# bupt-cist/vqa-playground-pytorch

Measured on AMD Instinct MI355X. Metric: VQA samples/sec (fwd+bwd), CoR2 batch 512, 36x2048 regions, higher is better.
Workload: dtype f32

## Files before the change

vqa_playground_pytorch_amd/csrc/bilinear_dw_rt.hip:

```cpp
#include <cstdlib>

#include "bilinear_folded.hpp"
#include "gemm_f32_rt.hpp"

namespace vqa {

namespace {

constexpr int kSpans = 5;
constexpr int kCols = 64 * kSpans;
typedef float f32x2 __attribute__((ext_vector_type(2)));
typedef unsigned int u32x2 __attribute__((__vector_size__(2 * sizeof(unsigned int))));

struct DwRtArgs {
  const float* g;
  const float* x;
  const float* h2;
  const float* w[2];
  const float* b[2];
  float* slab;
  float* dbslab;
  float* part;
  int B, N, L, H;
  int HB;
  int spl;
  unsigned long long* stamps;
};

template <int R, int NS, int D, int TUNE = 0>
__global__ __launch_bounds__(rt::kThreads, 1) void bilinear_dw_rt_kernel(DwRtArgs p) {
  using rt::f32x4;
  extern __shared__ __attribute__((aligned(16))) char smem_raw[];
  float* Ws = reinterpret_cast<float*>(smem_raw);
  const int tid = threadIdx.x, lane = tid & 63, r = lane & 15, gq = lane >> 4;
  const int wave = __builtin_amdgcn_readfirstlane(tid >> 6);
  const int eh = wave & 1, sl = wave >> 1;
  const int id = xcd_remap(blockIdx.x, gridDim.x);
  const int hb = id % p.HB, sg = id / p.HB;
  const int h0 = hb * 16;
  unsigned long long tk_in = 0;
  if constexpr ((TUNE & 4) != 0) tk_in = __builtin_amdgcn_s_memrealtime();
  const int slice = sg * 2 + sl;
  const int b_lo = min(slice * p.spl, p.B), b_hi = min(p.B, b_lo + p.spl);
  const int L = p.L, H = p.H, N = p.N;

  const rt::rsrc_t Gb = rt::make_rsrc(p.g, (size_t)p.B * N * H * 4);
  const rt::rsrc_t Xb = rt::make_rsrc(p.x, (size_t)p.B * N * L * 4);
  const rt::rsrc_t Hb = rt::make_rsrc(p.h2, (size_t)p.B * R * H * 4);
  const uint32_t offG = ((uint32_t)gq * (uint32_t)H + (uint32_t)min(h0 + r, H - 1)) * 4u;
  uint32_t offX[kSpans];
#pragma unroll
  for (int q = 0; q < kSpans; ++q) offX[q] = ((uint32_t)gq * (uint32_t)L + (uint32_t)(64 * q + 4 * r + 2 * eh)) * 4u;
  const uint32_t offH = (uint32_t)(h0 + 4 * gq) * 4u;
  const bool one_lane = (r == (L % 64) / 4) && (eh == (L % 4) / 2);

  f32x4 acc[R][kSpans][2];
#pragma unroll
  for (int rk = 0; rk < R; ++rk)
#pragma unroll
    for (int q = 0; q < kSpans; ++q)
#pragma unroll
      for (int e = 0; e < 2; ++e) acc[rk][q][e] = f32x4{0.f, 0.f, 0.f, 0.f};

  struct Step {
    float a;
    f32x2 xb[kSpans];
  };
  const int row_hi = b_hi * N;
  auto load_step = [&](Step& st, int row) {
    const uint32_t rw = (uint32_t)min(row, max(row_hi - 4, 0));
    st.a = rt::ldg4(Gb, offG, rw * (uint32_t)H * 4u);
#pragma unroll
    for (int q = 0; q < kSpans; ++q)
      st.xb[q] = __builtin_bit_cast(f32x2, __builtin_amdgcn_raw_buffer_load_b64(Xb, (int)offX[q], (int)(rw * (uint32_t)L * 4u), 0));
  };
  auto fix_ones = [&](Step& st) {
    const float v0 = st.xb[kSpans - 1][0], v1 = st.xb[kSpans - 1][1];
    st.xb[kSpans - 1][0] = one_lane ? 1.f : v0;
    st.xb[kSpans - 1][1] = one_lane ? 0.f : v1;
  };

  Step ring[D];
#pragma unroll
  for (int d = 0; d < D; ++d) load_step(ring[d], b_lo * N + 4 * d);
  f32x4 h2v[R];
#pragma unroll
  for (int rk = 0; rk < R; ++rk) h2v[rk] = rt::ldg16(Hb, offH, (uint32_t)((min(b_lo, p.B - 1) * R + rk) * H) * 4u);

  {
    const int hl = tid >> 4, c0 = (tid & 15) * 2;
    const int h = h0 + hl;
    f32x2 wv[R][kCols / 32];
    float bv[R];
    constexpr uint32_t kOut = 0x80000000u;
#pragma unroll
    for (int rk = 0; rk < R; ++rk) {
      const rt::rsrc_t Wb = rt::make_rsrc(p.w[rk], (size_t)H * L * 4);
      const rt::rsrc_t Bb = rt::make_rsrc(p.b[rk], (size_t)H * 4);
      bv[rk] = rt::ldg4(Bb, h < H ? (uint32_t)h * 4u : kOut, 0u);
#pragma unroll
      for (int k = 0; k < kCols / 32; ++k) {
        const int col = c0 + 32 * k;
        const uint32_t off = (h < H && col < L) ? ((uint32_t)h * (uint32_t)L + (uint32_t)col) * 4u : kOut;
        wv[rk][k] = __builtin_bit_cast(f32x2, __builtin_amdgcn_raw_buffer_load_b64(Wb, (int)off, 0, 0));
      }
    }
#pragma unroll
    for (int rk = 0; rk < R; ++rk)
#pragma unroll
      for (int k = 0; k < kCols / 32; ++k)
        if (c0 + 32 * k == L) wv[rk][k][0] = bv[rk];
#pragma unroll
    for (int rk = 0; rk < R; ++rk)
#pragma unroll
      for (int k = 0; k < kCols / 32; ++k)
        *reinterpret_cast<f32x2*>(Ws + (rk * 16 + hl) * kCols + c0 + 32 * k) = wv[rk][k];
  }
  __syncthreads();

  if (b_lo < b_hi) {

    f32x4 P[kSpans][2];
    unsigned long long cyc_steps = 0, cyc_fold = 0, tk0 = 0;
    if constexpr ((TUNE & 4) != 0) tk0 = __builtin_amdgcn_s_memrealtime();
    for (int b = b_lo; b < b_hi; ++b) {
      const int row0 = b * N;
      unsigned long long c0 = 0, c1 = 0;
      if constexpr ((TUNE & 4) != 0) c0 = __builtin_amdgcn_s_memtime();
      f32x4 h2n[R];
#pragma unroll
      for (int rk = 0; rk < R; ++rk) h2n[rk] = rt::ldg16(Hb, offH, (uint32_t)((min(b + 1, b_hi - 1) * R + rk) * H) * 4u);
#pragma unroll
      for (int s = 0; s < NS; ++s) {
        static_assert(NS % D == 0, "a ring slot must mean the same step in every sample");
        Step& st = ring[s % D];
        fix_ones(st);
#pragma unroll
        for (int q = 0; q < kSpans; ++q)
#pragma unroll
          for (int e = 0; e < 2; ++e)
            P[q][e] = __builtin_amdgcn_mfma_f32_16x16x4f32(st.a, st.xb[q][e], s == 0 ? f32x4{0.f, 0.f, 0.f, 0.f} : P[q][e], 0, 0, 0);
        load_step(ring[(s + D - 1) % D], row0 + 4 * (s - 1 + D));
        __builtin_amdgcn_sched_group_barrier(0x002, 2, 0);
        __builtin_amdgcn_sched_group_barrier(0x008, 1, 0);
#pragma unroll
        for (int t = 0; t < kSpans + 1; ++t) {
          __builtin_amdgcn_sched_group_barrier(0x020, 1, 0);
          __builtin_amdgcn_sched_group_barrier(0x008, 1, 0);
        }
        __builtin_amdgcn_sched_group_barrier(0x008, 2 * kSpans - 1 - (kSpans + 1), 0);
        __builtin_amdgcn_sched_barrier(0);
      }
      if constexpr ((TUNE & 4) != 0) {
        c1 = __builtin_amdgcn_s_memtime();
        cyc_steps += c1 - c0;
      }
      f32x4 dh[R];
#pragma unroll
      for (int rk = 0; rk < R; ++rk) dh[rk] = f32x4{0.f, 0.f, 0.f, 0.f};
#pragma unroll
      for (int q = 0; q < kSpans; ++q) {
        f32x2 wq[R][4];
#pragma unroll
        for (int rk = 0; rk < R; ++rk)
#pragma unroll
          for (int t = 0; t < 4; ++t)
            wq[rk][t] = *reinterpret_cast<const f32x2*>(Ws + (rk * 16 + 4 * gq + t) * kCols + 64 * q + 4 * r + 2 * eh);
#pragma unroll
        for (int e = 0; e < 2; ++e) {
          const f32x4 pv = P[q][e];
#pragma unroll
          for (int rk = 0; rk < R; ++rk) {
            acc[rk][q][e] += h2v[rk] * pv;
#pragma unroll
            for (int t = 0; t < 4; ++t) dh[rk][t] = fmaf(wq[rk][t][e], pv[t], dh[rk][t]);
          }
        }
      }
      {
        const int h = h0 + 4 * gq + (r & 3);
        const bool odd = (r & 1) != 0, hi = (r & 2) != 0;
#pragma unroll
        for (int rk = 0; rk < R; ++rk) {
          float k01 = odd ? dh[rk][1] : dh[rk][0], s01 = odd ? dh[rk][0] : dh[rk][1];
          float k23 = odd ? dh[rk][3] : dh[rk][2], s23 = odd ? dh[rk][2] : dh[rk][3];
          k01 += dpp_mov<0xB1>(s01);
          k23 += dpp_mov<0xB1>(s23);
          float v = hi ? k23 : k01;
          const float sv = hi ? k01 : k23;
          v += dpp_mov<0x4E>(sv);
          v += dpp_mov<0x124>(v);
          v += dpp_mov<0x128>(v);
          if (r < 4 && h < H) p.part[(size_t)eh * p.B * R * H + ((size_t)b * R + rk) * H + h] = v;
        }
      }
#pragma unroll
      for (int rk = 0; rk < R; ++rk) h2v[rk] = h2n[rk];
      if constexpr ((TUNE & 4) != 0) cyc_fold += __builtin_amdgcn_s_memtime() - c1;
    }
    if constexpr ((TUNE & 4) != 0) {
      if (lane == 0 && p.stamps != nullptr) {
        unsigned long long* st = p.stamps + (size_t)(blockIdx.x * 4 + wave) * 5;
        st[0] = cyc_steps;
        st[1] = cyc_fold;
        st[2] = __builtin_amdgcn_s_memrealtime() - tk0;
        st[3] = tk0 - tk_in;
      }
    }
  }

  constexpr int NBLK = R * kSpans * 2;
  f32x4* box = reinterpret_cast<f32x4*>(smem_raw) + (size_t)eh * NBLK * 64 + lane;
  __syncthreads();
  if (sl == 1) {
#pragma unroll
    for (int rk = 0; rk < R; ++rk)
#pragma unroll
      for (int q = 0; q < kSpans; ++q)
#pragma unroll
        for (int e = 0; e < 2; ++e) box[(size_t)((rk * kSpans + q) * 2 + e) * 64] = acc[rk][q][e];
  }
  __syncthreads();
  if (sl == 1) return;
#pragma unroll
  for (int rk = 0; rk < R; ++rk)
#pragma unroll
    for (int q = 0; q < kSpans; ++q)
#pragma unroll
      for (int e = 0; e < 2; ++e) acc[rk][q][e] += box[(size_t)((rk * kSpans + q) * 2 + e) * 64];

#pragma unroll
  for (int rk = 0; rk < R; ++rk) {
    float* __restrict__ dst = p.slab + ((size_t)sg * R + rk) * H * L;
    float* __restrict__ dbd = p.dbslab + ((size_t)sg * R + rk) * H;
#pragma unroll
    for (int q = 0; q < kSpans; ++q) {
      const int col = 64 * q + 4 * r + 2 * eh;
#pragma unroll
      for (int t = 0; t < 4; ++t) {
        const int h = h0 + 4 * gq + t;
        if (h >= H) continue;
        if (col + 1 < L)
          st2(dst + (size_t)h * L + col, make_float2(acc[rk][q][0][t], acc[rk][q][1][t]));
        else if (col == L)
          dbd[h] = acc[rk][q][0][t];
      }
    }
  }
  if constexpr ((TUNE & 4) != 0) {
    __builtin_amdgcn_s_waitcnt(0);
    if (lane == 0 && p.stamps != nullptr) p.stamps[(size_t)(blockIdx.x * 4 + wave) * 5 + 4] = __builtin_amdgcn_s_memrealtime() - tk_in;
  }
}

}

bool dw_rt_supported(int B, int N, int L, int H, int R, int ldx) {
  const bool off = vqa::option_is("VQA_K4_DW_RT", '0');
  return !off && (R == 1 || R == 2) && (N == 36 || N == 100) && L > 256 && L < kCols && ldx == L && L % 2 == 0 && H >= 16 &&
         B >= 64 && (size_t)B * N * H * 4 < (1ull << 32);
}

int dw_rt_launch(const float* g, const float* x, const float* h2, const float* const* w1, const float* const* b1, float* slab,
                 float* dbslab, float* part, int B, int N, int L, int H, int R, hipStream_t s) {
  DwRtArgs a{};
  a.g = g;
  a.x = x;
  a.h2 = h2;
  for (int r = 0; r < R; ++r) {
    a.w[r] = w1[r];
    a.b[r] = b1[r];
  }
  a.slab = slab;
  a.dbslab = dbslab;
  a.part = part;
  a.B = B;
  a.N = N;
  a.L = L;
  a.H = H;
  a.HB = (H + 15) / 16;
  a.spl = (B + 2 * kDwRtGroups - 1) / (2 * kDwRtGroups);
  const dim3 grid(a.HB * kDwRtGroups);
  const int tune = vqa::option("VQA_K4_DW_TUNE") ? std::atoi(vqa::option("VQA_K4_DW_TUNE")) : 0;
#define LAUNCH(R_, NS_)                                                                                         \
  {                                                                                                             \
     \
    const size_t lds_w = (size_t)R_ * 16 * kCols * 4, lds_b = (size_t)2 * R_ * kSpans * 2 * 64 * 16;            \
    const size_t lds = lds_w > lds_b ? lds_w : lds_b;                                                           \
    constexpr int D_ = NS_ == 9 ? 9 : 5;               \
    VQA_ENSURE_LDS((bilinear_dw_rt_kernel<R_, NS_, D_>), lds);                                                  \
    if (tune == 4 && R_ == 2 && NS_ == 9) {                                                                \
      static unsigned long long* st = nullptr;                                                                  \
      if (st == nullptr) (void)hipMalloc(&st, 1024 * 5 * 8);                                                    \
      a.stamps = st;                                                                                            \
      VQA_LAUNCH((bilinear_dw_rt_kernel<2, 9, 9, 4>), grid, dim3(rt::kThreads), lds, s, a);             \
      static int shown = 0;                                                                                     \
      if (++shown == 20) {                                                                                      \
        unsigned long long h[1024 * 5];                                                                         \
        (void)hipDeviceSynchronize();                                                                           \
        (void)hipMemcpy(h, st, sizeof(h), hipMemcpyDeviceToHost);                                               \
        double c0 = 0, c1 = 0, tk = 0, pro = 0, tot = 0, tkmax = 0, totmax = 0;                                 \
        int n0 = 0;                                                                                             \
        for (int i = 0; i < 1024; ++i) {                                                                        \
          c0 += h[5 * i]; c1 += h[5 * i + 1]; tk += h[5 * i + 2]; pro += h[5 * i + 3];                          \
          if ((double)h[5 * i + 2] > tkmax) tkmax = (double)h[5 * i + 2];                                       \
          if ((i & 3) < 2) { tot += h[5 * i + 4]; ++n0; if ((double)h[5 * i + 4] > totmax) totmax = (double)h[5 * i + 4]; } \
        }                                                                                                       \
        fprintf(stderr, "dw_rt stamps: steps %.0f cyc, fold %.0f cyc, loop %.2f us (max %.2f), prologue %.2f us, whole wave %.2f us (max %.2f)\n", \
                c0 / 1024, c1 / 1024, tk / 1024 / 100.0, tkmax / 100.0, pro / 1024 / 100.0, tot / n0 / 100.0, totmax / 100.0); \
      }                                                                                                         \
    }                                                                                                           \
    else                                                                                                        \
      VQA_LAUNCH((bilinear_dw_rt_kernel<R_, NS_, D_>), grid, dim3(rt::kThreads), lds, s, a);            \
  }
  if (R == 1) {
    if (N == 36) LAUNCH(1, 9) else LAUNCH(1, 25)
  } else {
    if (N == 36) LAUNCH(2, 9) else LAUNCH(2, 25)
  }
#undef LAUNCH
  return check_launch("lowrank_bilinear_fusion_folded_bwd (dW, register-tile)");
}

}
```

Baseline: 260,500.

## Software-pipeline dW fold of previous sample under MFMA steps of next sample

Adds a pipelined variant of the register-tile dW kernel that double-buffers the MFMA accumulators P. The VALU fold (acc update, dh reduction, DPP reduce and store) for sample b-1 is interleaved into the MFMA step loop of sample b using sched_group_barrier slots. The Ws loads are spread across steps the same way. The intent is to hide the serial fold phase behind matrix-core work. In exchange it doubles P register usage, which risks spills or lower scheduling freedom. The path is on by default and can be turned off with VQA_K4_DW_PIPE=0.

```diff
diff --git a/vqa_playground_pytorch_amd/csrc/bilinear_dw_rt.hip b/vqa_playground_pytorch_amd/csrc/bilinear_dw_rt.hip
--- a/vqa_playground_pytorch_amd/csrc/bilinear_dw_rt.hip
+++ b/vqa_playground_pytorch_amd/csrc/bilinear_dw_rt.hip
@@ -1,4 +1,5 @@
 #include <cstdlib>
+#include <utility>
 
 #include "bilinear_folded.hpp"
 #include "gemm_f32_rt.hpp"
@@ -9,8 +10,25 @@
 
 constexpr int kSpans = 5;
 constexpr int kCols = 64 * kSpans;
+constexpr int kDwFoldValu = 5;
 typedef float f32x2 __attribute__((ext_vector_type(2)));
 typedef unsigned int u32x2 __attribute__((__vector_size__(2 * sizeof(unsigned int))));
+
+template <class F, int... I>
+__device__ __forceinline__ void unrolled_seq(F&& f, std::integer_sequence<int, I...>) {
+  (f(std::integral_constant<int, I>{}), ...);
+}
+template <int N, class F>
+__device__ __forceinline__ void unrolled(F&& f) {
+  unrolled_seq(f, std::make_integer_sequence<int, N>{});
+}
+
+constexpr int wq_step(int q, int NS, int NU) { return (2 * q * NS / NU + NS - 1) % NS; }
+constexpr int wq_spans_at(int s, int NS, int NU, bool fold) {
+  int n = 0;
+  for (int q = 0; q < kSpans; ++q) n += (wq_step(q, NS, NU) == s && (fold || s == NS - 1)) ? 1 : 0;
+  return n;
+}
 
 struct DwRtArgs {
   const float* g;
@@ -27,7 +45,7 @@
   unsigned long long* stamps;
 };
 
-template <int R, int NS, int D, int TUNE = 0>
+template <int R, int NS, int D, int TUNE = 0, int FV = 0>
 __global__ __launch_bounds__(rt::kThreads, 1) void bilinear_dw_rt_kernel(DwRtArgs p) {
   using rt::f32x4;
   extern __shared__ __attribute__((aligned(16))) char smem_raw[];
@@ -120,68 +138,119 @@
 
   if (b_lo < b_hi) {
 
-    f32x4 P[kSpans][2];
     unsigned long long cyc_steps = 0, cyc_fold = 0, tk0 = 0;
     if constexpr ((TUNE & 4) != 0) tk0 = __builtin_amdgcn_s_memrealtime();
-    for (int b = b_lo; b < b_hi; ++b) {
-      const int row0 = b * N;
-      unsigned long long c0 = 0, c1 = 0;
-      if constexpr ((TUNE & 4) != 0) c0 = __builtin_amdgcn_s_memtime();
+    if constexpr (FV == 0) {
+      f32x4 P[kSpans][2];
+      for (int b = b_lo; b < b_hi; ++b) {
+        const int row0 = b * N;
+        unsigned long long c0 = 0, c1 = 0;
+        if constexpr ((TUNE & 4) != 0) c0 = __builtin_amdgcn_s_memtime();
+        f32x4 h2n[R];
+#pragma unroll
+        for (int rk = 0; rk < R; ++rk) h2n[rk] = rt::ldg16(Hb, offH, (uint32_t)((min(b + 1, b_hi - 1) * R + rk) * H) * 4u);
+#pragma unroll
+        for (int s = 0; s < NS; ++s) {
+          static_assert(NS % D == 0, "a ring slot must mean the same step in every sample");
+          Step& st = ring[s % D];
+          fix_ones(st);
+#pragma unroll
+          for (int q = 0; q < kSpans; ++q)
+#pragma unroll
+            for (int e = 0; e < 2; ++e)
+              P[q][e] = __builtin_amdgcn_mfma_f32_16x16x4f32(st.a, st.xb[q][e], s == 0 ? f32x4{0.f, 0.f, 0.f, 0.f} : P[q][e], 0, 0, 0);
+          load_step(ring[(s + D - 1) % D], row0 + 4 * (s - 1 + D));
+          __builtin_amdgcn_sched_group_barrier(0x002, 2, 0);
+          __builtin_amdgcn_sched_group_barrier(0x008, 1, 0);
+#pragma unroll
+          for (int t = 0; t < kSpans + 1; ++t) {
+            __builtin_amdgcn_sched_group_barrier(0x020, 1, 0);
+            __builtin_amdgcn_sched_group_barrier(0x008, 1, 0);
+          }
+          __builtin_amdgcn_sched_group_barrier(0x008, 2 * kSpans - 1 - (kSpans + 1), 0);
+          __builtin_amdgcn_sched_barrier(0);
+        }
+        if constexpr ((TUNE & 4) != 0) {
+          c1 = __builtin_amdgcn_s_memtime();
+          cyc_steps += c1 - c0;
+        }
+        f32x4 dh[R];
+#pragma unroll
+        for (int rk = 0; rk < R; ++rk) dh[rk] = f32x4{0.f, 0.f, 0.f, 0.f};
+#pragma unroll
+        for (int q = 0; q < kSpans; ++q) {
+          f32x2 wq[R][4];
+#pragma unroll
+          for (int rk = 0; rk < R; ++rk)
+#pragma unroll
+            for (int t = 0; t < 4; ++t)
+              wq[rk][t] = *reinterpret_cast<const f32x2*>(Ws + (rk * 16 + 4 * gq + t) * kCols + 64 * q + 4 * r + 2 * eh);
+#pragma unroll
+          for (int e = 0; e < 2; ++e) {
+            const f32x4 pv = P[q][e];
+#pragma unroll
+            for (int rk = 0; rk < R; ++rk) {
+              acc[rk][q][e] += h2v[rk] * pv;
+#pragma unroll
+              for (int t = 0; t < 4; ++t) dh[rk][t] = fmaf(wq[rk][t][e], pv[t], dh[rk][t]);
+            }
+          }
+        }
+        {
+          const int h = h0 + 4 * gq + (r & 3);
+          const bool odd = (r & 1) != 0, hi = (r & 2) != 0;
+#pragma unroll
+          for (int rk = 0; rk < R; ++rk) {
+            float k01 = odd ? dh[rk][1] : dh[rk][0], s01 = odd ? dh[rk][0] : dh[rk][1];
+            float k23 = odd ? dh[rk][3] : dh[rk][2], s23 = odd ? dh[rk][2] : dh[rk][3];
+            k01 += dpp_mov<0xB1>(s01);
+            k23 += dpp_mov<0xB1>(s23);
+            float v = hi ? k23 : k01;
+            const float sv = hi ? k01 : k23;
+            v += dpp_mov<0x4E>(sv);
+            v += dpp_mov<0x124>(v);
+            v += dpp_mov<0x128>(v);
+            if (r < 4 && h < H) p.part[(size_t)eh * p.B * R * H + ((size_t)b * R + rk) * H + h] = v;
+          }
+        }
+#pragma unroll
+        for (int rk = 0; rk < R; ++rk) h2v[rk] = h2n[rk];
+        if constexpr ((TUNE & 4) != 0) cyc_fold += __builtin_amdgcn_s_memtime() - c1;
+      }
+    } else {
+      f32x4 P[2][kSpans][2];
+      constexpr int NU = 2 * kSpans + R;
+      f32x2 wq[kSpans][R][4];
+      f32x4 dh[R];
       f32x4 h2n[R];
-#pragma unroll
-      for (int rk = 0; rk < R; ++rk) h2n[rk] = rt::ldg16(Hb, offH, (uint32_t)((min(b + 1, b_hi - 1) * R + rk) * H) * 4u);
-#pragma unroll
-      for (int s = 0; s < NS; ++s) {
-        static_assert(NS % D == 0, "a ring slot must mean the same step in every sample");
-        Step& st = ring[s % D];
-        fix_ones(st);
-#pragma unroll
-        for (int q = 0; q < kSpans; ++q)
-#pragma unroll
-          for (int e = 0; e < 2; ++e)
-            P[q][e] = __builtin_amdgcn_mfma_f32_16x16x4f32(st.a, st.xb[q][e], s == 0 ? f32x4{0.f, 0.f, 0.f, 0.f} : P[q][e], 0, 0, 0);
-        load_step(ring[(s + D - 1) % D], row0 + 4 * (s - 1 + D));
-        __builtin_amdgcn_sched_group_barrier(0x002, 2, 0);
-        __builtin_amdgcn_sched_group_barrier(0x008, 1, 0);
-#pragma unroll
-        for (int t = 0; t < kSpans + 1; ++t) {
-          __builtin_amdgcn_sched_group_barrier(0x020, 1, 0);
-          __builtin_amdgcn_sched_group_barrier(0x008, 1, 0);
-        }
-        __builtin_amdgcn_sched_group_barrier(0x008, 2 * kSpans - 1 - (kSpans + 1), 0);
-        __builtin_amdgcn_sched_barrier(0);
-      }
-      if constexpr ((TUNE & 4) != 0) {
-        c1 = __builtin_amdgcn_s_memtime();
-        cyc_steps += c1 - c0;
-      }
-      f32x4 dh[R];
-#pragma unroll
-      for (int rk = 0; rk < R; ++rk) dh[rk] = f32x4{0.f, 0.f, 0.f, 0.f};
-#pragma unroll
-      for (int q = 0; q < kSpans; ++q) {
-        f32x2 wq[R][4];
+      const rt::rsrc_t Db = rt::make_rsrc(p.part, (size_t)2 * p.B * R * H * 4);
+      const uint32_t offD = (r < 4 && h0 + 4 * gq + (r & 3) < H) ? (uint32_t)(((size_t)eh * p.B * R * H + h0 + 4 * gq + (r & 3)) * 4u) : 0x80000000u;
+      auto load_wq = [&](auto qc) __attribute__((always_inline)) {
+        constexpr int q = decltype(qc)::value;
 #pragma unroll
         for (int rk = 0; rk < R; ++rk)
 #pragma unroll
           for (int t = 0; t < 4; ++t)
-            wq[rk][t] = *reinterpret_cast<const f32x2*>(Ws + (rk * 16 + 4 * gq + t) * kCols + 64 * q + 4 * r + 2 * eh);
-#pragma unroll
-        for (int e = 0; e < 2; ++e) {
-          const f32x4 pv = P[q][e];
+            wq[q][rk][t] = *reinterpret_cast<const f32x2*>(Ws + (rk * 16 + 4 * gq + t) * kCols + 64 * q + 4 * r + 2 * eh);
+      };
+      auto fold_unit = [&](const f32x4 (&Pf)[kSpans][2], int bf, auto uc) __attribute__((always_inline)) {
+        constexpr int u = decltype(uc)::value;
+        if constexpr (u < 2 * kSpans) {
+          constexpr int q = u / 2, e = u % 2;
+          if constexpr (u == 0) {
+#pragma unroll
+            for (int rk = 0; rk < R; ++rk) dh[rk] = f32x4{0.f, 0.f, 0.f, 0.f};
+          }
+          const f32x4 pv = Pf[q][e];
 #pragma unroll
           for (int rk = 0; rk < R; ++rk) {
             acc[rk][q][e] += h2v[rk] * pv;
 #pragma unroll
-            for (int t = 0; t < 4; ++t) dh[rk][t] = fmaf(wq[rk][t][e], pv[t], dh[rk][t]);
-          }
-        }
-      }
-      {
-        const int h = h0 + 4 * gq + (r & 3);
-        const bool odd = (r & 1) != 0, hi = (r & 2) != 0;
-#pragma unroll
-        for (int rk = 0; rk < R; ++rk) {
+            for (int t = 0; t < 4; ++t) dh[rk][t] = fmaf(wq[q][rk][t][e], pv[t], dh[rk][t]);
+          }
+        } else {
+          constexpr int rk = u - 2 * kSpans;
+          const bool odd = (r & 1) != 0, hi = (r & 2) != 0;
           float k01 = odd ? dh[rk][1] : dh[rk][0], s01 = odd ? dh[rk][0] : dh[rk][1];
           float k23 = odd ? dh[rk][3] : dh[rk][2], s23 = odd ? dh[rk][2] : dh[rk][3];
           k01 += dpp_mov<0xB1>(s01);
@@ -191,12 +260,110 @@
           v += dpp_mov<0x4E>(sv);
           v += dpp_mov<0x124>(v);
           v += dpp_mov<0x128>(v);
-          if (r < 4 && h < H) p.part[(size_t)eh * p.B * R * H + ((size_t)b * R + rk) * H + h] = v;
-        }
-      }
-#pragma unroll
-      for (int rk = 0; rk < R; ++rk) h2v[rk] = h2n[rk];
-      if constexpr ((TUNE & 4) != 0) cyc_fold += __builtin_amdgcn_s_memtime() - c1;
+          __builtin_amdgcn_raw_buffer_store_b32(__builtin_bit_cast(unsigned int, v), Db, (int)offD, (int)((uint32_t)((bf * R + rk) * H) * 4u), 0);
+        }
+      };
+      auto fold_all = [&](const f32x4 (&Pf)[kSpans][2], int bf) __attribute__((always_inline)) {
+        unrolled<kSpans>([&](auto qc) __attribute__((always_inline)) {
+          constexpr int q = decltype(qc)::value;
+          load_wq(qc);
+          fold_unit(Pf, bf, std::integral_constant<int, 2 * q>{});
+          fold_unit(Pf, bf, std::integral_constant<int, 2 * q + 1>{});
+        });
+        unrolled<R>([&](auto rc) __attribute__((always_inline)) { fold_unit(Pf, bf, std::integral_constant<int, 2 * kSpans + decltype(rc)::value>{}); });
+      };
+
+      auto steps = [&](f32x4 (&Pc)[kSpans][2], const f32x4 (&Pf)[kSpans][2], int b, int bh, auto foldc) __attribute__((always_inline)) {
+        constexpr bool FOLD = decltype(foldc)::value;
+        const int row0 = b * N;
+#pragma unroll
+        for (int rk = 0; rk < R; ++rk) h2n[rk] = rt::ldg16(Hb, offH, (uint32_t)((bh * R + rk) * H) * 4u);
+        unrolled<NS>([&](auto sc) __attribute__((always_inline)) {
+          constexpr int s = decltype(sc)::value;
+          static_assert(NS % D == 0, "a ring slot must mean the same step in every sample");
+          Step& st = ring[s % D];
+          fix_ones(st);
+#pragma unroll
+          for (int q = 0; q < kSpans; ++q)
+#pragma unroll
+            for (int e = 0; e < 2; ++e)
+              Pc[q][e] = __builtin_amdgcn_mfma_f32_16x16x4f32(st.a, st.xb[q][e], s == 0 ? f32x4{0.f, 0.f, 0.f, 0.f} : Pc[q][e], 0, 0, 0);
+          load_step(ring[(s + D - 1) % D], row0 + 4 * (s - 1 + D));
+          constexpr int u_lo = FOLD ? (s * NU + NS - 1) / NS : 0, u_hi = FOLD ? ((s + 1) * NU + NS - 1) / NS : 0;
+          constexpr int nwq = wq_spans_at(s, NS, NU, FOLD);
+          if constexpr (nwq > 0) {
+            unrolled<kSpans>([&](auto qc) __attribute__((always_inline)) {
+              if constexpr (wq_step(decltype(qc)::value, NS, NU) == s) load_wq(qc);
+            });
+          }
+          unrolled<u_hi - u_lo>([&](auto ic) __attribute__((always_inline)) {
+            constexpr int u = u_lo + decltype(ic)::value;
+            fold_unit(Pf, b - 1, std::integral_constant<int, u>{});
+            if constexpr (u < 2 * kSpans) {
+#pragma unroll
+              for (int rk = 0; rk < R; ++rk) {
+                f32x4 a = acc[rk][u / 2][u % 2], d = dh[rk];
+                asm volatile("" : "+v"(a[0]), "+v"(a[1]), "+v"(a[2]), "+v"(a[3]), "+v"(d[0]), "+v"(d[1]), "+v"(d[2]), "+v"(d[3]));
+                acc[rk][u / 2][u % 2] = a;
+                dh[rk] = d;
+              }
+            }
+          });
+          __builtin_amdgcn_sched_group_barrier(0x002, 2, 0);
+          __builtin_amdgcn_sched_group_barrier(0x008, 1, 0);
+#pragma unroll
+          for (int t = 0; t < kSpans + 1; ++t) {
+            __builtin_amdgcn_sched_group_barrier(0x020, 1, 0);
+            if constexpr (nwq > 0)
+              if (t == 0) __builtin_amdgcn_sched_group_barrier(0x100, 4 * R * nwq, 0);
+            if constexpr (FOLD) __builtin_amdgcn_sched_group_barrier(0x002, FV, 0);
+            __builtin_amdgcn_sched_group_barrier(0x008, 1, 0);
+          }
+          if constexpr (FOLD) {
+#pragma unroll
+            for (int t = 0; t < 2 * kSpans - 1 - (kSpans + 1); ++t) {
+              __builtin_amdgcn_sched_group_barrier(0x002, FV, 0);
+              __builtin_amdgcn_sched_group_barrier(0x008, 1, 0);
+            }
+          } else {
+            __builtin_amdgcn_sched_group_barrier(0x008, 2 * kSpans - 1 - (kSpans + 1), 0);
+          }
+          __builtin_amdgcn_sched_barrier(0);
+        });
+      };
+      auto rotate_h2 = [&]() __attribute__((always_inline)) {
+#pragma unroll
+        for (int rk = 0; rk < R; ++rk) h2v[rk] = h2n[rk];
+      };
+      auto stamp = [&](unsigned long long& sum, unsigned long long& c) __attribute__((always_inline)) {
+        if constexpr ((TUNE & 4) != 0) {
+          const unsigned long long now = __builtin_amdgcn_s_memtime();
+          sum += now - c;
+          c = now;
+        }
+      };
+      unsigned long long c = 0;
+      if constexpr ((TUNE & 4) != 0) c = __builtin_amdgcn_s_memtime();
+
+      steps(P[0], P[1], b_lo, b_lo, std::false_type{});
+      rotate_h2();
+      int b = b_lo + 1;
+      for (; b + 1 < b_hi; b += 2) {
+        steps(P[1], P[0], b, b, std::true_type{});
+        rotate_h2();
+        steps(P[0], P[1], b + 1, b + 1, std::true_type{});
+        rotate_h2();
+      }
+      if (b < b_hi) {
+        steps(P[1], P[0], b, b, std::true_type{});
+        rotate_h2();
+        stamp(cyc_steps, c);
+        fold_all(P[1], b);
+      } else {
+        stamp(cyc_steps, c);
+        fold_all(P[0], b - 1);
+      }
+      stamp(cyc_fold, c);
     }
     if constexpr ((TUNE & 4) != 0) {
       if (lane == 0 && p.stamps != nullptr) {
@@ -281,19 +448,22 @@
   a.HB = (H + 15) / 16;
   a.spl = (B + 2 * kDwRtGroups - 1) / (2 * kDwRtGroups);
   const dim3 grid(a.HB * kDwRtGroups);
+  const bool pipe = !vqa::option_is("VQA_K4_DW_PIPE", '0');
   const int tune = vqa::option("VQA_K4_DW_TUNE") ? std::atoi(vqa::option("VQA_K4_DW_TUNE")) : 0;
-#define LAUNCH(R_, NS_)                                                                                         \
+#define LAUNCH(R_, NS_, PIPE_)                                                                                      \
   {                                                                                                             \
      \
     const size_t lds_w = (size_t)R_ * 16 * kCols * 4, lds_b = (size_t)2 * R_ * kSpans * 2 * 64 * 16;            \
     const size_t lds = lds_w > lds_b ? lds_w : lds_b;                                                           \
     constexpr int D_ = NS_ == 9 ? 9 : 5;               \
-    VQA_ENSURE_LDS((bilinear_dw_rt_kernel<R_, NS_, D_>), lds);                                                  \
+    constexpr int FV_ = PIPE_ ? kDwFoldValu : 0;                                                                \
+    VQA_ENSURE_LDS((bilinear_dw_rt_kernel<R_, NS_, D_, 0, FV_>), lds);                                          \
     if (tune == 4 && R_ == 2 && NS_ == 9) {                                                                \
       static unsigned long long* st = nullptr;                                                                  \
       if (st == nullptr) (void)hipMalloc(&st, 1024 * 5 * 8);                                                    \
       a.stamps = st;                                                                                            \
-      VQA_LAUNCH((bilinear_dw_rt_kernel<2, 9, 9, 4>), grid, dim3(rt::kThreads), lds, s, a);             \
+      VQA_ENSURE_LDS((bilinear_dw_rt_kernel<2, 9, 9, 4, FV_>), lds);                                            \
+      VQA_LAUNCH((bilinear_dw_rt_kernel<2, 9, 9, 4, FV_>), grid, dim3(rt::kThreads), lds, s, a);                \
       static int shown = 0;                                                                                     \
       if (++shown == 20) {                                                                                      \
         unsigned long long h[1024 * 5];                                                                         \
@@ -311,13 +481,16 @@
       }                                                                                                         \
     }                                                                                                           \
     else                                                                                                        \
-      VQA_LAUNCH((bilinear_dw_rt_kernel<R_, NS_, D_>), grid, dim3(rt::kThreads), lds, s, a);            \
-  }
-  if (R == 1) {
-    if (N == 36) LAUNCH(1, 9) else LAUNCH(1, 25)
-  } else {
-    if (N == 36) LAUNCH(2, 9) else LAUNCH(2, 25)
-  }
+      VQA_LAUNCH((bilinear_dw_rt_kernel<R_, NS_, D_, 0, FV_>), grid, dim3(rt::kThreads), lds, s, a);            \
+  }
+#define LAUNCH_R(R_)                                                     \
+  if (pipe) {                                                            \
+    if (N == 36) LAUNCH(R_, 9, true) else LAUNCH(R_, 25, true)           \
+  } else {                                                               \
+    if (N == 36) LAUNCH(R_, 9, false) else LAUNCH(R_, 25, false)         \
+  }
+  if (R == 1) LAUNCH_R(1) else LAUNCH_R(2)
+#undef LAUNCH_R
 #undef LAUNCH
   return check_launch("lowrank_bilinear_fusion_folded_bwd (dW, register-tile)");
 }
```

Result: no change. 263,100, median of 6 (+1.0%).
